# crowdbotp/socialways

Measured on AMD Instinct MI355X. Metric: GAN train steps/sec (256 scenes x 8 agents x 8+12 T per GPU step; fp32; social block on), higher is better.
Workload: dtype f32; 1 GPU; m1: 256 scenes x 8 agents x (8 obs + 12 pred) per GPU step = reference --batch-size 2048; use_social=True, n_unrolling_steps=1, info loss on; full=False, global_batch_scenes=256, parallelism=dp1, steps_per_graph_launch=32, settle_steps=992, rehearsal_regions=2, step_alg_bytes=5527040, inputs=z drawn on the host every step

## Files before the change

### socialways_amd/csrc/sw_disc.hip

```cpp
#include "../../include/socialways_hip.h"
#include "sw_lstm_dev.h"
#include "sw_wgrad.h"
#include "sw_wgrad_dev.h"
#include <cstdlib>
#ifdef SW_PHASE_STAMPS
__device__ long long sw_disc_stamps[16];
#define SW_STAMP(k) do { __builtin_amdgcn_sched_barrier(0); long long _t = clock64(); if (blockIdx.x == 0 && threadIdx.x == 0) sw_disc_stamps[k] += _t - _tprev; _tprev = _t; __builtin_amdgcn_sched_barrier(0); } while (0)
#define SW_STAMP_INIT long long _tprev = clock64()
extern "C" int sw_debug_disc_stamps(long long* out, int reset) {
  if (reset) { long long z[16] = {0}; return (int)hipMemcpyToSymbol(HIP_SYMBOL(sw_disc_stamps), z, sizeof(z)); }
  return (int)hipMemcpyFromSymbol(out, HIP_SYMBOL(sw_disc_stamps), 16 * sizeof(long long));
}
#else
#define SW_STAMP(k)
#define SW_STAMP_INIT
#endif

#define SW_DSTAMP(k) SW_STAMP(k)
#define SW_DSTAMP_INIT SW_STAMP_INIT
#include "sw_disc_dev.h"

__global__ __launch_bounds__(SW_THREADS, 2) void disc_fwd_kernel(
    const float* __restrict__ obsv, int To, int x_mode, const float* __restrict__ pred_a,
    const float* __restrict__ pred_b, int nb, const float* __restrict__ d_w, int B, int Tp, float* __restrict__ label_a, float* __restrict__ label_b,
// ... 231 lines not shown
  const bool live = (a0 + ln) < B;
  const int K4 = 4 * Tp, ldp = U.ldp;
  float* hw = smem + U.hw - F.of0;
  float* hwT = smem + U.hwT - T.of0T;

  float xpre[2][4];
  disc_xpre_load(xpre, pred_a, pred_b, a0, B, K4, ldp);
  const float tg0 = gl.targets[gl.t0], tg1 = gl.targets[gl.t1];
  const float z0 = gl.z[(size_t)b * SW_Z], z1 = gl.z[(size_t)b * SW_Z + 1];
  LstmW W;
  if (!obs_pre) disc_obs_operands(W, d_w, O, dimg);
  if (w_snap)
    for (int i = blockIdx.x * SW_THREADS + threadIdx.x; i < O.n; i += gridDim.x * SW_THREADS) w_snap[i] = d_w[i];
  disc_stage_heads(hw, F, d_w, O, K4, true);
  disc_stage_headT(hwT, T, true, nullptr, O, K4, dimg, false);
#pragma unroll
  for (int kk = 0; kk < 2; ++kk)
    disc_xpre_put(xpre, kk == 1, smem + U.x + kk * 16 * ldp, dsave + ds.px + (size_t)kk * B * K4, a0, B, K4, ldp);
  f32x4 c = {0.f, 0.f, 0.f, 0.f}, h = {0.f, 0.f, 0.f, 0.f};
  disc_seed_h(hbuf, obs_pre, dsave + ds.act, To, B, b);
  sw_barrier();
  const bool reg8 = !obs_pre && To == 8;
  f32x4 sg[8][4], sc[8];
  if (reg8) {
    float xa, xq;
    obs_x4_load(obsv, b, 0, 8, lg, xa, xq);
    asm volatile("" : "+v"(xa), "+v"(xq));
    float* hrow_g = dsave + ds.act + (size_t)b * 384 + 320 + u0 + 4 * lg;
    float* xrow = dsave + ds.x4s + (size_t)b * 4 + lg;
#pragma unroll
    for (int t = 0; t < 8; ++t) {
      const float xb = xa - (lg >= 2 ? xq : 0.f);
      obs_x4_load(obsv, b, t + 1 < 8 ? t + 1 : 7, 8, lg, xa, xq);
      lstm_cell(W, xb, &hbuf[(t & 1) * 16 * SW_HLD + ln * SW_HLD + 4 * lg], sg[t], c, h);
      sc[t] = c;
      st4(&hbuf[((t + 1) & 1) * 16 * SW_HLD + ln * SW_HLD + u0 + 4 * lg], h);
      st4g(hrow_g, h);
      *xrow = xb;
      hrow_g += (size_t)B * 384;
      xrow += (size_t)B * 4;
      sw_barrier();
      asm volatile("" : "+v"(xa), "+v"(xq));
    }
  } else if (!obs_pre) {
    lstm_obs_loop<0, true>(W, hbuf, obsv, To, B, b, c, h, dsave + ds.act, dsave + ds.x4s);
  }
  const float* hlast = &hbuf[(To & 1) * 16 * SW_HLD];

  const f32x4 o1reg = disc_obs_fc(hw, F, hlast, smem + U.o1, dsave + ds.o1 + (size_t)b * 32, live, smem + U.both, 2);
  float* xb_ = smem + U.x + br * 16 * ldp;
  float* q1_ = smem + U.q1 + br * 16 * LD32;
  float* both_ = smem + U.both + br * 16 * LD64;
  float* c1_ = smem + U.c1 + br * 16 * LD32;
  float* l1_ = smem + U.l1 + br * 16 * LD32;
  const size_t kb = (size_t)br * B + b;
  f32x4 q1reg, c1reg, l1reg;
  {
    const int m0 = 16 * wp;
    f32x4 acc = ld4(smem + U.bias + 2 * 32 + m0 + 4 * lg);
    acc = tile_mm_rt(hw + F.pe0 + (m0 + ln) * ldp + 4 * lg, xb_ + ln * ldp + 4 * lg, (ldp - 4) / 16, acc);
#pragma unroll
    for (int r = 0; r < 4; ++r) acc[r] = sw_lrelu(acc[r]);
    q1reg = acc;
    st4(q1_ + ln * LD32 + m0 + 4 * lg, acc);
    if (live) st4(dsave + ds.q1 + kb * 32 + m0 + 4 * lg, acc);
  }
  sw_barrier();
// ... 530 lines not shown
```

### socialways_amd/csrc/sw_lstm.hip

```cpp
#include "../../include/socialways_hip.h"
#include "sw_lstm_dev.h"
#include <cstdlib>

template <int XMODE, bool ACT, bool Y, bool X4S>
__global__ __launch_bounds__(SW_THREADS) void enc_lstm_fwd_kernel(
    const float* __restrict__ x, const float* __restrict__ enc_w, const float* __restrict__ h0,
    const float* __restrict__ c0, int B, int T, float* __restrict__ hT, float* __restrict__ cT,
    float* __restrict__ y, float* __restrict__ act, float* __restrict__ x4s, int t0, const float* __restrict__ aux_src,
    float* __restrict__ aux_dst, long long aux_n, const float* __restrict__ gimg) {
  const int tiles = (B + SW_TILE - 1) / SW_TILE;
  const int extra = (int)gridDim.x - tiles;
  if ((int)blockIdx.x < extra) {
    const long long n4 = aux_n >> 2, stride = (long long)extra * SW_THREADS;
    long long i = (long long)blockIdx.x * SW_THREADS + threadIdx.x;
    for (; i + 3 * stride < n4; i += 4 * stride) {
      const f32x4 v0 = ld4(aux_src + 4 * i), v1 = ld4(aux_src + 4 * (i + stride));
      const f32x4 v2 = ld4(aux_src + 4 * (i + 2 * stride)), v3 = ld4(aux_src + 4 * (i + 3 * stride));
      st4(aux_dst + 4 * i, v0);
      st4(aux_dst + 4 * (i + stride), v1);
      st4(aux_dst + 4 * (i + 2 * stride), v2);
      st4(aux_dst + 4 * (i + 3 * stride), v3);
    }
    for (; i < n4; i += stride) st4(aux_dst + 4 * i, ld4(aux_src + 4 * i));
    return;
  }
  constexpr int HS = ACT ? SW_ALD : SW_HLD, HO = ACT ? 320 : 0;
  __shared__ __attribute__((aligned(16))) float hbuf[2][SW_TILE * HS];
  __shared__ __attribute__((aligned(16))) float wx_lds[256 * 4];
  __shared__ __attribute__((aligned(16))) float bx_lds[256];
  const int lane = sw_lane(), wave = sw_wave(), ln = lane & 15, lg = lane >> 4;
  const int u0 = wave * 16;
  const int a0 = ((int)blockIdx.x - extra) * SW_TILE;
  const int b = min(a0 + ln, B - 1);
  LstmW W;
  if (gimg) {
    lstm_load_img(W, gimg, wave, lane);
  } else {
    lstm_load_whh(W, enc_w + swp::ENC_WHH, u0, ln, lg);
    lstm_prep_rows(enc_w + swp::ENC_EMB_W, enc_w + swp::ENC_EMB_B, enc_w + swp::ENC_WIH, enc_w + swp::ENC_BIH,
                   enc_w + swp::ENC_BHH, true, wx_lds, bx_lds);
  }
  f32x4 c = {0.f, 0.f, 0.f, 0.f}, h = {0.f, 0.f, 0.f, 0.f};
  if (h0) h = ld4(h0 + (size_t)b * 64 + u0 + 4 * lg);
  if (c0) c = ld4(c0 + (size_t)b * 64 + u0 + 4 * lg);
  st4(&hbuf[0][ln * HS + HO + u0 + 4 * lg], h);
  sw_barrier();
  if (!gimg) lstm_load_wx(W, wx_lds, bx_lds, u0, ln, lg);

  float xa, xq = 0.f;
  auto load_x = [&](int t) {
    if constexpr (XMODE == 0) obs_x4_load(x, b, t, T, lg, xa, xq);
    else xa = x[((size_t)b * T + t) * 4 + lg];
  };
  load_x(0);
  asm volatile("" : "+v"(xa), "+v"(xq));
  float* yrow = Y ? y + (size_t)b * T * 64 + u0 + 4 * lg : nullptr;
  float* xrow = X4S ? x4s + ((size_t)t0 * B + b) * 4 + lg : nullptr;
  for (int t = 0; t < T; ++t) {
    const float xb = XMODE == 0 ? xa - (lg >= 2 ? xq : 0.f) : xa;
    load_x(min(t + 1, T - 1));
    f32x4 gate[4];
    lstm_cell(W, xb, &hbuf[t & 1][ln * HS + HO + 4 * lg], gate, c, h);
    if constexpr (ACT) lstm_put_act_tile(hbuf[(t + 1) & 1], gate, c, h, ln, lg, u0);
    else st4(&hbuf[(t + 1) & 1][ln * HS + u0 + 4 * lg], h);
    if constexpr (Y) {
      st4(yrow, h);
      yrow += 64;
    }
    if constexpr (X4S) {
      *xrow = xb;
      xrow += (size_t)B * 4;
    }
    sw_barrier();
    if constexpr (ACT) lstm_store_act_tile(hbuf[(t + 1) & 1], act + (size_t)(t0 + t) * B * 384, a0, B, wave, lane);
    asm volatile("" : "+v"(xa), "+v"(xq));
  }
  st4(hT + (size_t)b * 64 + u0 + 4 * lg, h);
  st4(cT + (size_t)b * 64 + u0 + 4 * lg, c);
}

__global__ __launch_bounds__(512) void enc_lstm_fwd8_kernel(
    const float* __restrict__ x, const float* __restrict__ h0, const float* __restrict__ c0, int B, int T,
    float* __restrict__ hT, float* __restrict__ cT, float* __restrict__ act, float* __restrict__ x4s, int t0,
    const float* __restrict__ aux_src, float* __restrict__ aux_dst, long long aux_n, const float* __restrict__ gimg) {
  const int tiles = (B + SW_TILE - 1) / SW_TILE;
  const int extra = (int)gridDim.x - tiles;
  if ((int)blockIdx.x < extra) {
    const long long n4 = aux_n >> 2, stride = (long long)extra * 512;
    long long i = (long long)blockIdx.x * 512 + threadIdx.x;
    for (; i + stride < n4; i += 2 * stride) {
      const f32x4 v0 = ld4(aux_src + 4 * i), v1 = ld4(aux_src + 4 * (i + stride));
      st4(aux_dst + 4 * i, v0);
      st4(aux_dst + 4 * (i + stride), v1);
    }
    for (; i < n4; i += stride) st4(aux_dst + 4 * i, ld4(aux_src + 4 * i));
    return;
  }
  __shared__ __attribute__((aligned(16))) float hbuf[2][SW_TILE * SW_ALD];
  const int lane = sw_lane(), wave = sw_wave(), ln = lane & 15, lg = lane >> 4;
  const int ub = 8 * wave + 2 * lg;
  const int a0 = ((int)blockIdx.x - extra) * SW_TILE;
  const int b = min(a0 + ln, B - 1);
  f32x4 whh[2][4], bias[2];
  float wx[2];
#pragma unroll
  for (int tl = 0; tl < 2; ++tl) {
#pragma unroll
    for (int j = 0; j < 4; ++j) whh[tl][j] = ld4(gimg + swimg::OP_WHH8 + ((((size_t)wave * 2 + tl) * 4 + j) * 64 + lane) * 4);
    const int rowA = (2 * tl + ((ln & 3) >> 1)) * 64 + 8 * wave + 2 * (ln >> 2) + (ln & 1);
    wx[tl] = gimg[swimg::WX + rowA * 4 + lg];
#pragma unroll
    for (int r = 0; r < 4; ++r) bias[tl][r] = gimg[swimg::BX + (2 * tl + (r >> 1)) * 64 + ub + (r & 1)];
  }
  float2 c = {0.f, 0.f}, h = {0.f, 0.f};
  if (h0) h = *reinterpret_cast<const float2*>(h0 + (size_t)b * 64 + ub);
  if (c0) c = *reinterpret_cast<const float2*>(c0 + (size_t)b * 64 + ub);
  *reinterpret_cast<float2*>(&hbuf[0][ln * SW_ALD + 320 + ub]) = h;
  sw_barrier();
  float xa, xq = 0.f;
  obs_x4_load(x, b, 0, T, lg, xa, xq);
  asm volatile("" : "+v"(xa), "+v"(xq));
  float* xrow = x4s + ((size_t)t0 * B + b) * 4 + lg;
  for (int t = 0; t < T; ++t) {
    const float xb = xa - (lg >= 2 ? xq : 0.f);
    obs_x4_load(x, b, min(t + 1, T - 1), T, lg, xa, xq);
    const float* hrow = &hbuf[t & 1][ln * SW_ALD + 320 + 4 * lg];
    f32x4 bq[4];
#pragma unroll
    for (int j = 0; j < 4; ++j) bq[j] = ld4(hrow + 16 * j);
    f32x4 acc0 = SW_MFMA(wx[0], xb, bias[0]), acc1 = SW_MFMA(wx[1], xb, bias[1]);
#pragma unroll
    for (int j = 0; j < 4; ++j)
#pragma unroll
      for (int r = 0; r < 4; ++r) {
        acc0 = SW_MFMA(whh[0][j][r], bq[j][r], acc0);
        acc1 = SW_MFMA(whh[1][j][r], bq[j][r], acc1);
      }
    float2 gi, gf, gg, go;
#pragma unroll
    for (int e = 0; e < 2; ++e) {
      const float i_ = sw_sigmoid(acc0[e]), f_ = sw_sigmoid(acc0[2 + e]), g_ = sw_tanh(acc1[e]), o_ = sw_sigmoid(acc1[2 + e]);
      const float cp = e ? c.y : c.x;
      const float cn = fmaf(f_, cp, i_ * g_);
      const float hn = o_ * sw_tanh(cn);
      if (e) { gi.y = i_; gf.y = f_; gg.y = g_; go.y = o_; c.y = cn; h.y = hn; }
      else   { gi.x = i_; gf.x = f_; gg.x = g_; go.x = o_; c.x = cn; h.x = hn; }
    }
    float* row = &hbuf[(t + 1) & 1][ln * SW_ALD + ub];
    *reinterpret_cast<float2*>(row) = gi;
    *reinterpret_cast<float2*>(row + 64) = gf;
    *reinterpret_cast<float2*>(row + 128) = gg;
    *reinterpret_cast<float2*>(row + 192) = go;
    *reinterpret_cast<float2*>(row + 256) = c;
    *reinterpret_cast<float2*>(row + 320) = h;
    *xrow = xb;
    xrow += (size_t)B * 4;
    sw_barrier();
    {
      float* rows_t = act + (size_t)(t0 + t) * B * 384;
#pragma unroll
      for (int k = 0; k < 3; ++k) {
        const int f = k * 512 + (int)threadIdx.x, a = f / 96, c4 = f - a * 96;
        const f32x4 v = ld4(&hbuf[(t + 1) & 1][a * SW_ALD + 4 * c4]);
        st4g(rows_t + (size_t)min(a0 + a, B - 1) * 384 + 4 * c4, v);
      }
    }
    asm volatile("" : "+v"(xa), "+v"(xq));
  }
  *reinterpret_cast<float2*>(hT + (size_t)b * 64 + ub) = h;
  *reinterpret_cast<float2*>(cT + (size_t)b * 64 + ub) = c;
}

template <bool DY>
__global__ __launch_bounds__(SW_THREADS) void enc_lstm_bwd_kernel(
    const float* __restrict__ whh, const float* __restrict__ act, const float* __restrict__ c0,
    const float* __restrict__ dhT, const float* __restrict__ dcT, const float* __restrict__ dy, int B, int T,
    int t0, float* __restrict__ dgates, float* __restrict__ dh0, float* __restrict__ dc0, const float* __restrict__ gimg,
    const float* __restrict__ aux_src, float* __restrict__ aux_dst, const float* __restrict__ aux_mask, long long aux_n) {
  if (sw_aux_masked_copy(B, aux_src, aux_dst, aux_mask, aux_n)) return;
  __shared__ __attribute__((aligned(16))) float dgbuf[2][SW_TILE * SW_GLD];
  const int lane = sw_lane(), wave = sw_wave(), ln = lane & 15, lg = lane >> 4;
  const int u0 = wave * 16;
  const int a0 = blockIdx.x * SW_TILE;
  const int b = min(a0 + ln, B - 1);
  LstmWT W;
  lstm_load_whhT(W, gimg, swimg::OP_WHHT, whh, wave, lane);
  const float* act_b = act + ((size_t)t0 * B + b) * 384 + u0 + 4 * lg;
  f32x4 dh = ld4(dhT ? dhT + (size_t)b * 64 + u0 + 4 * lg : act_b);
  f32x4 dc = ld4(dcT ? dcT + (size_t)b * 64 + u0 + 4 * lg : act_b);
  if (!dhT) dh = f32x4{0.f, 0.f, 0.f, 0.f};
  if (!dcT) dc = f32x4{0.f, 0.f, 0.f, 0.f};
  const float* cstart = t0 > 0 ? act_b - (size_t)B * 384 + 256 : c0 ? c0 + (size_t)b * 64 + u0 + 4 * lg : nullptr;
  const LstmBptt S{act_b, cstart, dgbuf[0], dgates + ((size_t)t0 * B + a0) * 256, nullptr, a0, B};
  const float* dyp = DY ? dy + ((size_t)b * T + T - 1) * 64 + u0 + 4 * lg : nullptr;
  lstm_bptt_rows<true>(W, S, T, dh, dc, [&](f32x4& d) {
    if constexpr (DY) {
      d += ld4(dyp);
      dyp -= 64;
    }
  });
  if (dh0) st4(dh0 + (size_t)b * 64 + u0 + 4 * lg, dh);
// ... 156 lines not shown
```

### socialways_amd/csrc/sw_lstm_dev.h

```cpp
#pragma once
#include "sw_common.h"

#define SW_HLD 68
#define SW_GLD 260

struct LstmW {
  f32x4 whh[4][4];
  float wx[4];
  f32x4 bias[4];
};

__device__ __forceinline__ void lstm_prep_rows(const float* We, const float* be, const float* Wih,
                                               const float* bih, const float* bhh, bool composed,
                                               float* wx_lds, float* bx_lds) {
  int row = threadIdx.x;
  if (composed) {
    f32x4 w[16];
    const float* wr = Wih + (size_t)row * 64;
#pragma unroll
    for (int e = 0; e < 16; ++e) w[e] = ld4(wr + 4 * e);
    float a0 = 0.f, a1 = 0.f, a2 = 0.f, a3 = 0.f, ab = 0.f;
#pragma unroll
    for (int e = 0; e < 16; ++e) {
      f32x4 bq = ld4(be + 4 * e);
#pragma unroll
      for (int q = 0; q < 4; ++q) {
        f32x4 em = ld4(We + (4 * e + q) * 4);
        a0 = fmaf(w[e][q], em[0], a0);
        a1 = fmaf(w[e][q], em[1], a1);
        a2 = fmaf(w[e][q], em[2], a2);
        a3 = fmaf(w[e][q], em[3], a3);
        ab = fmaf(w[e][q], bq[q], ab);
      }
// ... 10 lines not shown
    wx_lds[row * 4 + 2] = w[2];
    wx_lds[row * 4 + 3] = w[3];
    bx_lds[row] = bih[row] + bhh[row];
  }
}

__device__ __forceinline__ void lstm_load_whh(LstmW& W, const float* Whh, int u0, int ln, int lg) {
#pragma unroll
  for (int g = 0; g < 4; ++g) {
    const float* wr = Whh + (size_t)(g * 64 + u0 + ln) * 64 + 4 * lg;
#pragma unroll
    for (int j = 0; j < 4; ++j) W.whh[g][j] = ld4(wr + 16 * j);
  }
}
__device__ __forceinline__ void lstm_load_wx(LstmW& W, const float* wx_lds, const float* bx_lds, int u0, int ln, int lg) {
#pragma unroll
  for (int g = 0; g < 4; ++g) {
    W.wx[g] = wx_lds[(g * 64 + u0 + ln) * 4 + lg];
    W.bias[g] = ld4(bx_lds + g * 64 + u0 + 4 * lg);
  }
}

__device__ __forceinline__ void lstm_load_img(LstmW& W, const float* __restrict__ gimg, int wave, int lane) {
  const int ln = lane & 15, lg = lane >> 4, u0 = wave * 16;
#pragma unroll
  for (int g = 0; g < 4; ++g) {
#pragma unroll
    for (int j = 0; j < 4; ++j) W.whh[g][j] = ld4(gimg + swimg::OP_WHH + ((((size_t)4 * g + wave) * 4 + j) * 64 + lane) * 4);
    W.wx[g] = gimg[swimg::WX + (g * 64 + u0 + ln) * 4 + lg];
    W.bias[g] = ld4(gimg + swimg::BX + g * 64 + u0 + 4 * lg);
  }
}

template <int NB>
__device__ __forceinline__ void lstm_products(const LstmW& W, const float (&xb)[NB], const float* const (&hrow)[NB],
                                              f32x4 (&acc)[NB][4]) {
  f32x4 b[NB][4];
#pragma unroll
  for (int k = 0; k < NB; ++k) {
#pragma unroll
    for (int j = 0; j < 4; ++j) b[k][j] = ld4(hrow[k] + 16 * j);
#pragma unroll
    for (int g = 0; g < 4; ++g) acc[k][g] = SW_MFMA(W.wx[g], xb[k], W.bias[g]);
  }
#pragma unroll
  for (int j = 0; j < 4; ++j) {
#pragma unroll
    for (int r = 0; r < 4; ++r) {
#pragma unroll
      for (int g = 0; g < 4; ++g) {
#pragma unroll
        for (int k = 0; k < NB; ++k) acc[k][g] = SW_MFMA(W.whh[g][j][r], b[k][j][r], acc[k][g]);
      }
    }
  }
}

__device__ __forceinline__ void lstm_gates(const f32x4 acc[4], f32x4 gate[4], f32x4& c, f32x4& h) {
#pragma unroll
  for (int r = 0; r < 4; ++r) {
    float i = sw_sigmoid(acc[0][r]);
    float f = sw_sigmoid(acc[1][r]);
    float g = sw_tanh(acc[2][r]);
    float o = sw_sigmoid(acc[3][r]);
    float cn = fmaf(f, c[r], i * g);
    gate[0][r] = i;
    gate[1][r] = f;
    gate[2][r] = g;
    gate[3][r] = o;
    c[r] = cn;
    h[r] = o * sw_tanh(cn);
  }
}

template <int NB>
__device__ __forceinline__ void lstm_cell(const LstmW& W, const float (&xb)[NB], const float* const (&hrow)[NB],
                                          f32x4 (&gate)[NB][4], f32x4 (&c)[NB], f32x4 (&h)[NB]) {
  f32x4 acc[NB][4];
  lstm_products<NB>(W, xb, hrow, acc);
#pragma unroll
  for (int k = 0; k < NB; ++k) lstm_gates(acc[k], gate[k], c[k], h[k]);
}
__device__ __forceinline__ void lstm_cell(const LstmW& W, float xb, const float* hrow, f32x4 gate[4],
                                          f32x4& c, f32x4& h) {
  f32x4 acc[1][4];
  lstm_products<1>(W, {xb}, {hrow}, acc);
  lstm_gates(acc[0], gate, c, h);
}

__device__ __forceinline__ void lstm_cell_bwd(const f32x4 gate[4], f32x4 ct, f32x4 cprev, f32x4 dh,
                                              f32x4& dc, f32x4 dgate[4]) {
#pragma unroll
  for (int r = 0; r < 4; ++r) {
    float i = gate[0][r], f = gate[1][r], g = gate[2][r], o = gate[3][r];
    float tc = sw_tanh(ct[r]);
    float d_o = dh[r] * tc;
    float dct = fmaf(dh[r] * o, 1.0f - tc * tc, dc[r]);
    dgate[0][r] = dct * g * i * (1.0f - i);
    dgate[1][r] = dct * cprev[r] * f * (1.0f - f);
    dgate[2][r] = dct * i * (1.0f - g * g);
    dgate[3][r] = d_o * o * (1.0f - o);
    dc[r] = dct * f;
  }
}

__device__ __forceinline__ void lstm_store_dgates_tile(const float* dgtile, float* __restrict__ rows ,
                                                       float* __restrict__ trash, int a0, int B, int wave, int lane) {
#pragma unroll
  for (int q = 0; q < 4; ++q) {
    const int a = 4 * wave + q;
    const f32x4 v = ld4(dgtile + a * SW_GLD + 4 * lane);
    float* dst = (a0 + a < B) ? rows + (size_t)a * 256 + 4 * lane
                 : trash      ? trash + a * 256 + 4 * lane
                              : rows + (size_t)(B - 1 - a0) * 256 + 4 * lane;
    st4g(dst, v);
  }
}

#define SW_ALD 388
// ... 116 lines not shown
    pre(dh);
  }
  lstm_bptt_step<false, false, DH0>(W, S, 0, gate, ct, cprev, dh, dc, stamp);
  stamp(11);
}

__device__ __forceinline__ void obs_x4_load(const float* pos, int b, int t, int T, int comp, float& a, float& q) {
  const float* p = pos + (size_t)b * T * 2;
  const int c = comp & 1, tt = t == 0 ? 1 : t;
  const bool vel = comp >= 2;
  a = p[(vel ? tt : t) * 2 + c];
  q = p[(vel ? tt - 1 : t) * 2 + c];
}
__device__ __forceinline__ float obs_x4(const float* pos, int b, int t, int T, int comp) {
  float a, q;
  obs_x4_load(pos, b, t, T, comp, a, q);
  return a - (comp >= 2 ? q : 0.f);
}

template <int XMODE, bool SAVE>
__device__ __forceinline__ void lstm_obs_loop(const LstmW& W, float* hbuf, const float* __restrict__ x, int T, int B, int b,
                                              f32x4& c, f32x4& h, float* __restrict__ act, float* __restrict__ x4s) {
  const int lane = sw_lane(), wave = sw_wave(), ln = lane & 15, lg = lane >> 4;
  const int u0 = wave * 16;
  float xa, xq = 0.f;
  auto load_x = [&](int t) {
    if constexpr (XMODE == 0) obs_x4_load(x, b, t, T, lg, xa, xq);
    else xa = x[((size_t)b * T + t) * 4 + lg];
  };
  load_x(0);
  asm volatile("" : "+v"(xa), "+v"(xq));
  float* arow = SAVE ? act + (size_t)b * 384 + u0 + 4 * lg : nullptr;
  float* xrow = SAVE ? x4s + (size_t)b * 4 + lg : nullptr;
  for (int t = 0; t < T; ++t) {
    const float xb = XMODE == 0 ? xa - (lg >= 2 ? xq : 0.f) : xa;
    load_x(min(t + 1, T - 1));
    f32x4 gate[4];
    lstm_cell(W, xb, &hbuf[(t & 1) * 16 * SW_HLD + ln * SW_HLD + 4 * lg], gate, c, h);
    st4(&hbuf[((t + 1) & 1) * 16 * SW_HLD + ln * SW_HLD + u0 + 4 * lg], h);
    if constexpr (SAVE) {
#pragma unroll
      for (int g = 0; g < 4; ++g) st4g(arow + g * 64, gate[g]);
      st4g(arow + 256, c);
      st4g(arow + 320, h);
      *xrow = xb;
      arow += (size_t)B * 384;
      xrow += (size_t)B * 4;
    }
    sw_barrier();
    asm volatile("" : "+v"(xa), "+v"(xq));
  }
}

__device__ __forceinline__ int obs_start(const int* __restrict__ obs_len, int b, int T, int xmode) {
  const int n = obs_len ? min(max(obs_len[b], xmode == 0 ? 2 : 1), T) : T;
  return T - n;
}
__device__ __forceinline__ void obs_x4_load_from(const float* pos, int b, int t, int s, int T, int comp, float& a, float& q) {
  const float* p = pos + (size_t)b * T * 2;
  const int c = comp & 1, te = max(t, s), tt = te == s ? s + 1 : te;
  const bool vel = comp >= 2;
  a = p[(vel ? tt : te) * 2 + c];
  q = p[(vel ? tt - 1 : te) * 2 + c];
}
template <int XMODE>
__device__ __forceinline__ void lstm_obs_loop_ragged(const LstmW& W, float* hbuf, const float* __restrict__ x, int T, int b, int s,
                                                     f32x4& c, f32x4& h) {
  const int lane = sw_lane(), wave = sw_wave(), ln = lane & 15, lg = lane >> 4;
  const int u0 = wave * 16;
  float xa, xq = 0.f;
  auto load_x = [&](int t) {
    if constexpr (XMODE == 0) obs_x4_load_from(x, b, t, s, T, lg, xa, xq);
    else xa = x[((size_t)b * T + max(t, s)) * 4 + lg];
  };
  load_x(0);
  asm volatile("" : "+v"(xa), "+v"(xq));
  for (int t = 0; t < T; ++t) {
    const float xb = XMODE == 0 ? xa - (lg >= 2 ? xq : 0.f) : xa;
    load_x(min(t + 1, T - 1));
    f32x4 gate[4];
    lstm_cell(W, xb, &hbuf[(t & 1) * 16 * SW_HLD + ln * SW_HLD + 4 * lg], gate, c, h);
    const bool on = t >= s;
#pragma unroll
    for (int r = 0; r < 4; ++r) {
// ... 29 lines not shown
```

### socialways_amd/csrc/sw_wgrad.hip

```cpp
#include "../../include/socialways_hip.h"
#include "sw_common.h"
#include "sw_wgrad.h"
#include "sw_wgrad_dev.h"
#include <stdlib.h>

__host__ __device__ inline int wg_grid_jobs(int total_jobs) { return (total_jobs + 31) & ~31; }
#ifdef SW_WG_STAMP
__device__ unsigned long long g_wg_stamps[4 * 4096];
extern "C" int sw_debug_wg_stamps(unsigned long long* host, int n) {
  return hipMemcpyFromSymbol(host, HIP_SYMBOL(g_wg_stamps), sizeof(unsigned long long) * (size_t)n) == hipSuccess ? 0 : -1;
}
#endif
__global__ __launch_bounds__(SW_THREADS, 2) void wgrad_partial_kernel(WgBatch batch, float* __restrict__ ws,
                                                                      const float* __restrict__ adam_step, double beta1,
                                                                      double beta2, float* __restrict__ bc_out) {
  __shared__ __attribute__((aligned(16))) float red[SW_WG_RED_FLOATS];
  if ((int)blockIdx.x >= wg_grid_jobs(batch.total_jobs)) {
    if (threadIdx.x == 0) {
      float bc1, bc2s;
      wg_adam_bc_compute(adam_step, beta1, beta2, bc1, bc2s);
      bc_out[0] = bc1;
      bc_out[1] = bc2s;
    }
    return;
// ... 67 lines not shown
  }
  float s = 0.f;
  float s1 = 0.f, s2 = 0.f, s3 = 0.f;
  int q = sub;
  for (; q + 3 * SW_WG_RSUB < P.nsplit; q += 4 * SW_WG_RSUB) {
    s += src[(size_t)q * stride];
    s1 += src[(size_t)(q + SW_WG_RSUB) * stride];
    s2 += src[(size_t)(q + 2 * SW_WG_RSUB) * stride];
    s3 += src[(size_t)(q + 3 * SW_WG_RSUB) * stride];
  }
  for (; q < P.nsplit; q += SW_WG_RSUB) s += src[(size_t)q * stride];
  s = (s + s1) + (s2 + s3);
#pragma unroll
  for (int o = SW_WG_REL; o < 64; o <<= 1) s += __shfl_xor(s, o);
  float bc1 = 1.f, bc2s = 1.f;
  if (ad.w) wg_adam_bc(ad, bc1, bc2s);
  if (!live || sub != 0) return;
  const float g = P.accumulate ? old1 + s : s;
  *dst = g;
  if (ad.w) wg_adam_fin(ad, a1, bc1, bc2s, g);
  if (dst2) {
    const float g2 = P.accumulate ? old2 + s : s;
    *dst2 = g2;
    if (ad.w) wg_adam_fin(ad, a2, bc1, bc2s, g2);
  }
}

bool wg_shape_ok(int N, int K) {
  for (int n0 = 0; n0 < N; n0 += 64)
    if (!wg_tiles(N - n0 < 64 ? N - n0 : 64, false)) return false;
  return K == 0 || wg_tiles(K, true) != 0;
}

int wg_add(WgBatch& b, const float* delta, int ldd, const float* act, int lda, int R, int N, int K, float* dW,
           int ldw, float* db, float* db2, int accumulate) {
  if (N > 256 || (ldd & 3) || (lda & 3)) return SW_ESHAPE;
  if ((long long)R * ldd >= (1LL << 31) || (long long)R * lda >= (1LL << 31)) return SW_ESHAPE;
  if (K < 1) return SW_ESHAPE;
  const int Nfull = N > 64 && (N & 63) && (N & 63) <= 32 && b.np + 2 * ((K + 63) / 64) <= SW_WG_MAXP ? (N & ~63) : N;
  for (int n0 = 0; n0 < N; n0 = (n0 == 0 ? Nfull : N)) {
    const int Nseg = n0 == 0 ? Nfull : N - Nfull;
    for (int c0 = 0; c0 < K; c0 += 64) {
      if (b.np >= SW_WG_MAXP) return SW_ESHAPE;
      const int c1 = c0 + 64 < K ? c0 + 64 : K;
      const bool has_ones = db && c1 == K;
      WgProblem& P = b.p[b.np++];
      P.delta = delta + n0; P.ldd = ldd; P.act = act + c0; P.lda = lda;
      P.R = R; P.N = Nseg; P.K = c1 - c0; P.ones = has_ones ? 1 : 0;
      P.dW = dW + (size_t)n0 * ldw + c0; P.ldw = ldw; P.db = has_ones ? db + n0 : nullptr;
      P.db2 = has_ones && db2 ? db2 + n0 : nullptr;
      P.accumulate = accumulate;
      P.pre = 0;
      P.act2 = nullptr; P.dW2 = nullptr; P.lda2 = P.ldw2 = P.K2 = P.row0 = 0;
      if (!wg_shape_ok(Nseg, P.K)) return SW_ESHAPE;
      P.nbn = (Nseg + 15) / 16;
      P.nbk = P.K > 0 ? wg_tiles(P.K, true) : 1;
    }
  }
  return SW_OK;
}

int wg_add_tail(WgBatch& b, const float* delta, int ldd, const float* act, int lda, int R, int N, int K, float* dW,
                int ldw, const float* act2, int lda2, int K2, float* dW2, int ldw2, int row0, float* db, float* db2,
                int accumulate) {
  if (N > 256 || (ldd & 3) || (lda & 3) || (lda2 & 3) || K != 64 || K2 != 4 || b.np >= SW_WG_MAXP)
    return SW_ESHAPE;
  if ((long long)R * ldd >= (1LL << 31) || (long long)R * lda >= (1LL << 31) || (long long)R * lda2 >= (1LL << 31)) return SW_ESHAPE;
  WgProblem& P = b.p[b.np++];
  P.delta = delta; P.ldd = ldd; P.act = act; P.lda = lda; P.R = R; P.N = N; P.K = K; P.ones = db ? 1 : 0;
  P.dW = dW; P.ldw = ldw; P.db = db; P.db2 = db ? db2 : nullptr; P.accumulate = accumulate; P.pre = 0;
  P.act2 = act2; P.lda2 = lda2; P.K2 = K2; P.dW2 = dW2; P.ldw2 = ldw2; P.row0 = row0;
  if (!wg_shape_ok(N, K)) return SW_ESHAPE;
  P.nbn = (N + 15) / 16;
  P.nbk = 4;
  return SW_OK;
}

int wg_add_pre(WgBatch& b, int N, int K, float* dW, int ldw, float* db, int nslices) {
  if (b.np >= SW_WG_MAXP || N < 1 || K < 1 || !db || nslices < 1) return SW_ESHAPE;
  WgProblem& P = b.p[b.np++];
  P.delta = nullptr; P.act = nullptr; P.ldd = P.lda = 0; P.R = 0;
  P.N = N; P.K = K; P.ones = 1; P.dW = dW; P.ldw = ldw; P.db = db; P.db2 = nullptr; P.accumulate = 0;
  P.nbn = (N + 15) / 16; P.nbk = (K + 1 + 15) / 16;
  P.act2 = nullptr; P.dW2 = nullptr; P.lda2 = P.ldw2 = P.K2 = P.row0 = 0;
  P.pre = nslices;
  b.top_reserved += (size_t)nslices * N * (K + 1);
  if (b.top_reserved > SW_WG_WS_FLOATS) return SW_ESHAPE;
  P.ws_off = SW_WG_WS_FLOATS - b.top_reserved;
  return SW_OK;
}

#ifndef SW_WG_GROUP_C0
#define SW_WG_GROUP_C0 256.0
#endif
#ifndef SW_WG_ROUND_UP
#define SW_WG_ROUND_UP 0.75
#endif
static double wg_cost(const WgProblem& P) {
  double c = 0;
  for (int n0 = 0; n0 < P.N; n0 += 64) {
// ... 121 lines not shown
```

### socialways_amd/csrc/sw_wgrad_dev.h

```cpp
#pragma once
#include <type_traits>
#include "sw_common.h"
#include "sw_wgrad.h"
#ifndef SW_WG_DEPTH
#define SW_WG_DEPTH 4
#endif
#ifndef SW_WG_DEPTH5
#define SW_WG_DEPTH5 2
#endif
#ifndef SW_WG_DEPTH_TAIL
#define SW_WG_DEPTH_TAIL SW_WG_DEPTH
#endif

#define SW_WG_RLD 69

template <int NV>
__device__ __forceinline__ void wg_ldv(float (&v)[NV], const float* p) {
  if constexpr (NV == 4) {
    const f32x4 q = *reinterpret_cast<const f32x4*>(p);
    v[0] = q[0]; v[1] = q[1]; v[2] = q[2]; v[3] = q[3];
  } else if constexpr (NV == 3) {
    struct __attribute__((packed, aligned(4))) P3 { float a, b, c; };
    const P3 q = *reinterpret_cast<const P3*>(p);
    v[0] = q.a; v[1] = q.b; v[2] = q.c;
  } else if constexpr (NV == 2) {
    const float2 q = *reinterpret_cast<const float2*>(p);
    v[0] = q.x; v[1] = q.y;
  } else {
    v[0] = p[0];
  }
}

__host__ __device__ inline int wg_tiles(int n, bool allow3) {
  if (n <= 16) return 1;
  for (int t = (n + 15) >> 4; t <= 4; ++t)
    if ((t != 3 || allow3) && n % t == 0) return t;
  return 0;
}

template <int NA, int KR, int K2, int ONES, int DSCALE = 1>
__device__ __forceinline__ void wg_run(const float* __restrict__ dbase, const float* __restrict__ abase, int ldd, int lda,
                                       int rbeg, int rend, int rmax, int acol, int bcol, int lg, int ln,
                                       float* __restrict__ mine,
                                       const float* __restrict__ abase2, int lda2, int row0, int xoff) {
  constexpr int KT = KR, XC = K2 + ONES;
  f32x4 acc[NA][KT];
#pragma unroll
  for (int i = 0; i < NA; ++i) {
#pragma unroll
    for (int kt = 0; kt < KT; ++kt) acc[i][kt] = f32x4{0.f, 0.f, 0.f, 0.f};
  }
  float xacc[NA][XC > 0 ? XC : 1];
#pragma unroll
  for (int i = 0; i < NA; ++i) {
#pragma unroll
    for (int c = 0; c < (XC > 0 ? XC : 1); ++c) xacc[i][c] = 0.f;
  }
  constexpr int DEPTH = (K2 > 0 ? SW_WG_DEPTH_TAIL : SW_WG_DEPTH) * DSCALE;
  float a[DEPTH][NA], b[DEPTH][KT];
  f32x4 xq[DEPTH];
  auto load = [&](int r0, float (&av)[NA], float (&bv)[KT], f32x4& xv) {
    const int rc = min(r0 + lg, rmax);
    wg_ldv<NA>(av, dbase + (unsigned)(rc * ldd + acol));
    if constexpr (K2 > 0) {
      wg_ldv<KR>(bv, abase + (unsigned)(max(rc, row0) * lda + bcol));
      xv = ld4(abase2 + (unsigned)(rc * lda2));
    } else {
      wg_ldv<KR>(bv, abase + (unsigned)(rc * lda + bcol));
    }
  };
#pragma unroll
  for (int q = 0; q < DEPTH - 1; ++q) load(rbeg + 4 * q, a[q], b[q], xq[q]);
  for (int r = rbeg; r < rend; r += 4 * DEPTH) {
#pragma unroll
    for (int q = 0; q < DEPTH; ++q) {
      load(r + 4 * (q + DEPTH - 1), a[(q + DEPTH - 1) % DEPTH], b[(q + DEPTH - 1) % DEPTH], xq[(q + DEPTH - 1) % DEPTH]);
      asm volatile("" ::: "memory");
#pragma unroll
      for (int i = 0; i < NA; ++i) asm volatile("" : "+v"(a[q][i]));
#pragma unroll
      for (int kt = 0; kt < KT; ++kt) asm volatile("" : "+v"(b[q][kt]));
      if constexpr (K2 > 0) asm volatile("" : "+v"(xq[q]));
      const int rr = r + 4 * q + lg;
      const float rs = rr < rend ? 1.0f : 0.0f;
      float av[NA], bv[KT];
#pragma unroll
      for (int i = 0; i < NA; ++i) av[i] = a[q][i] * rs;
      if constexpr (K2 > 0) {
        const float rs0 = rr >= row0 ? 1.0f : 0.0f;
#pragma unroll
        for (int kt = 0; kt < KR; ++kt) bv[kt] = b[q][kt] * rs0;
      } else {
#pragma unroll
        for (int kt = 0; kt < KR; ++kt) bv[kt] = b[q][kt];
      }
#pragma unroll
      for (int i = 0; i < NA; ++i) {
#pragma unroll
        for (int kt = 0; kt < KT; ++kt) {
          acc[i][kt] = SW_MFMA(av[i], bv[kt], acc[i][kt]);
        }
      }
#pragma unroll
      for (int i = 0; i < NA; ++i) {
        if constexpr (K2 > 0) {
#pragma unroll
          for (int c = 0; c < K2; ++c) xacc[i][c] = fmaf(av[i], xq[q][c], xacc[i][c]);
        }
        if constexpr (ONES) xacc[i][K2] += av[i];
      }
    }
  }
#pragma unroll
  for (int i = 0; i < NA; ++i) {
#pragma unroll
    for (int kt = 0; kt < KT; ++kt) {
#pragma unroll
      for (int r = 0; r < 4; ++r) {
        const int orow = NA * (4 * lg + r) + i;
        if (KR * ln + kt < xoff) mine[orow * SW_WG_RLD + KR * ln + kt] = acc[i][kt][r];
      }
    }
  }
  if constexpr (XC > 0) {
#pragma unroll
    for (int i = 0; i < NA; ++i) {
#pragma unroll
      for (int c = 0; c < XC; ++c) {
        float v = xacc[i][c];
        v += __shfl_xor(v, 16);
        v += __shfl_xor(v, 32);
        if (lg == 0) mine[(NA * ln + i) * SW_WG_RLD + xoff + c] = v;
      }
    }
  }
}

#define SW_WG_RED_FLOATS (4 * 64 * SW_WG_RLD)
template <int DSCALE = 1>
__device__ __forceinline__ void wg_job(const WgBatch& batch, float* __restrict__ ws, int job, float* red) {
  const int lane = sw_lane(), wave = sw_wave(), ln = lane & 15, lg = lane >> 4;
  int p = 0;
#pragma unroll 1
  while (p + 1 < batch.np && job >= batch.job0s[p + 1]) ++p;
  const WgProblem& P = batch.p[p];
  const int j = job - P.job0;
  const int NB = (P.N + 63) >> 6;
  const int sg = j / NB, nb = j - sg * NB;
  const int s = sg * 4 + wave;
  const int N = P.N, K = P.K, Kc = P.K + P.K2 + P.ones;
  const int n0 = nb * 64;
  const int Nb = min(64, N - n0);
  const int NA = wg_tiles(Nb, false);
  const int KR = K > 0 ? wg_tiles(K, true) : 1;
  const int nsub = P.nsplit * 4;
  const int rows_per = (((P.R + nsub - 1) / nsub) + 3) & ~3;
  const int rbeg = min(P.R, s * rows_per);
  const int rend = min(P.R, rbeg + rows_per);
  const int acol = n0 + max(0, min(NA * ln, Nb - NA));
  const int bcol = max(0, min(KR * ln, K - KR));
  float* mine = red + wave * 64 * SW_WG_RLD;
#define WG_CASE(na, kr, k2, on)                                                                                     \
  case ((na * 8 + kr) * 2 + (k2 ? 1 : 0)) * 2 + on:                                                                 \
    wg_run<na, kr, k2, on, DSCALE>(P.delta, P.act, P.ldd, P.lda, rbeg, rend, P.R - 1, acol, bcol, lg, ln,              \
                                   mine, P.act2 ? P.act2 : P.delta, P.act2 ? P.lda2 : P.ldd, P.row0, K);            \
    break;
#define WG_CASES(na)                                                                                                \
  WG_CASE(na, 1, 0, 0) WG_CASE(na, 2, 0, 0) WG_CASE(na, 3, 0, 0) WG_CASE(na, 4, 0, 0)                               \
  WG_CASE(na, 1, 0, 1) WG_CASE(na, 2, 0, 1) WG_CASE(na, 3, 0, 1) WG_CASE(na, 4, 0, 1)                               \
  WG_CASE(na, 4, 4, 0) WG_CASE(na, 4, 4, 1)
  switch (((NA * 8 + KR) * 2 + (P.K2 ? 1 : 0)) * 2 + (P.ones ? 1 : 0)) {
    WG_CASES(1) WG_CASES(2) WG_CASES(4)
  }
#undef WG_CASES
#undef WG_CASE
  sw_barrier();
  float* out = ws + P.ws_off + (size_t)sg * N * Kc;
  const int rows = min(64, N - n0), cols = min(SW_WG_RLD, Kc);
  const int dq = SW_THREADS / cols, dr = SW_THREADS - dq * cols;
  int rr = threadIdx.x / cols, cc = threadIdx.x - rr * cols;
  const float* r0 = red, *r1 = red + 64 * SW_WG_RLD, *r2 = red + 2 * 64 * SW_WG_RLD, *r3 = red + 3 * 64 * SW_WG_RLD;
  for (int e = threadIdx.x; e < rows * cols; e += SW_THREADS) {
    const int o = rr * SW_WG_RLD + cc;
    const float v = (r0[o] + r1[o]) + (r2[o] + r3[o]);
    out[(size_t)(n0 + rr) * Kc + cc] = v;
    cc += dr;
    rr += dq;
    if (cc >= cols) {
      cc -= cols;
      ++rr;
    }
  }
}
```

Baseline: 2753 steps/s.

## Skip recurrent matmul at zero initial state and use buffer loads in wgrad

The first LSTM step of the encoder, discriminator and generic obs loops now skips the hidden-state LDS reads and the W_hh MFMA chain when the initial hidden state is known to be zero. Separately, the weight-gradient inner loop now uses raw buffer loads with per-range descriptors. Out-of-range rows read as zero, which removes the per-row clamp and masking multiplies. The host-side span checks are updated to fit the descriptor byte limits. The risk is correctness at range edges, since masking now relies on the buffer bounds and on row0 handling through the descriptor base.

```diff
diff --git a/socialways_amd/csrc/sw_disc.hip b/socialways_amd/csrc/sw_disc.hip
--- a/socialways_amd/csrc/sw_disc.hip
+++ b/socialways_amd/csrc/sw_disc.hip
@@ -287,7 +287,9 @@
     for (int t = 0; t < 8; ++t) {
       const float xb = xa - (lg >= 2 ? xq : 0.f);
       obs_x4_load(obsv, b, t + 1 < 8 ? t + 1 : 7, 8, lg, xa, xq);
-      lstm_cell(W, xb, &hbuf[(t & 1) * 16 * SW_HLD + ln * SW_HLD + 4 * lg], sg[t], c, h);
+      const float* hrow = &hbuf[(t & 1) * 16 * SW_HLD + ln * SW_HLD + 4 * lg];
+      if (t == 0) lstm_cell<false>(W, xb, hrow, sg[t], c, h);
+      else lstm_cell(W, xb, hrow, sg[t], c, h);
       sc[t] = c;
       st4(&hbuf[((t + 1) & 1) * 16 * SW_HLD + ln * SW_HLD + u0 + 4 * lg], h);
       st4g(hrow_g, h);
diff --git a/socialways_amd/csrc/sw_lstm.hip b/socialways_amd/csrc/sw_lstm.hip
--- a/socialways_amd/csrc/sw_lstm.hip
+++ b/socialways_amd/csrc/sw_lstm.hip
@@ -56,11 +56,11 @@
   asm volatile("" : "+v"(xa), "+v"(xq));
   float* yrow = Y ? y + (size_t)b * T * 64 + u0 + 4 * lg : nullptr;
   float* xrow = X4S ? x4s + ((size_t)t0 * B + b) * 4 + lg : nullptr;
-  for (int t = 0; t < T; ++t) {
+  auto step = [&](int t, auto hp) {
     const float xb = XMODE == 0 ? xa - (lg >= 2 ? xq : 0.f) : xa;
     load_x(min(t + 1, T - 1));
     f32x4 gate[4];
-    lstm_cell(W, xb, &hbuf[t & 1][ln * HS + HO + 4 * lg], gate, c, h);
+    lstm_cell<decltype(hp)::value>(W, xb, &hbuf[t & 1][ln * HS + HO + 4 * lg], gate, c, h);
     if constexpr (ACT) lstm_put_act_tile(hbuf[(t + 1) & 1], gate, c, h, ln, lg, u0);
     else st4(&hbuf[(t + 1) & 1][ln * HS + u0 + 4 * lg], h);
     if constexpr (Y) {
@@ -74,7 +74,10 @@
     sw_barrier();
     if constexpr (ACT) lstm_store_act_tile(hbuf[(t + 1) & 1], act + (size_t)(t0 + t) * B * 384, a0, B, wave, lane);
     asm volatile("" : "+v"(xa), "+v"(xq));
-  }
+  };
+  if (h0) step(0, std::true_type{});
+  else step(0, std::false_type{});
+  for (int t = 1; t < T; ++t) step(t, std::true_type{});
   st4(hT + (size_t)b * 64 + u0 + 4 * lg, h);
   st4(cT + (size_t)b * 64 + u0 + 4 * lg, c);
 }
@@ -121,21 +124,23 @@
   obs_x4_load(x, b, 0, T, lg, xa, xq);
   asm volatile("" : "+v"(xa), "+v"(xq));
   float* xrow = x4s + ((size_t)t0 * B + b) * 4 + lg;
-  for (int t = 0; t < T; ++t) {
+  auto step = [&](int t, auto hp) {
     const float xb = xa - (lg >= 2 ? xq : 0.f);
     obs_x4_load(x, b, min(t + 1, T - 1), T, lg, xa, xq);
-    const float* hrow = &hbuf[t & 1][ln * SW_ALD + 320 + 4 * lg];
-    f32x4 bq[4];
-#pragma unroll
-    for (int j = 0; j < 4; ++j) bq[j] = ld4(hrow + 16 * j);
     f32x4 acc0 = SW_MFMA(wx[0], xb, bias[0]), acc1 = SW_MFMA(wx[1], xb, bias[1]);
-#pragma unroll
-    for (int j = 0; j < 4; ++j)
-#pragma unroll
-      for (int r = 0; r < 4; ++r) {
-        acc0 = SW_MFMA(whh[0][j][r], bq[j][r], acc0);
-        acc1 = SW_MFMA(whh[1][j][r], bq[j][r], acc1);
-      }
+    if constexpr (decltype(hp)::value) {
+      const float* hrow = &hbuf[t & 1][ln * SW_ALD + 320 + 4 * lg];
+      f32x4 bq[4];
+#pragma unroll
+      for (int j = 0; j < 4; ++j) bq[j] = ld4(hrow + 16 * j);
+#pragma unroll
+      for (int j = 0; j < 4; ++j)
+#pragma unroll
+        for (int r = 0; r < 4; ++r) {
+          acc0 = SW_MFMA(whh[0][j][r], bq[j][r], acc0);
+          acc1 = SW_MFMA(whh[1][j][r], bq[j][r], acc1);
+        }
+    }
     float2 gi, gf, gg, go;
 #pragma unroll
     for (int e = 0; e < 2; ++e) {
@@ -166,7 +171,10 @@
       }
     }
     asm volatile("" : "+v"(xa), "+v"(xq));
-  }
+  };
+  if (h0) step(0, std::true_type{});
+  else step(0, std::false_type{});
+  for (int t = 1; t < T; ++t) step(t, std::true_type{});
   *reinterpret_cast<float2*>(hT + (size_t)b * 64 + ub) = h;
   *reinterpret_cast<float2*>(cT + (size_t)b * 64 + ub) = c;
 }
diff --git a/socialways_amd/csrc/sw_lstm_dev.h b/socialways_amd/csrc/sw_lstm_dev.h
--- a/socialways_amd/csrc/sw_lstm_dev.h
+++ b/socialways_amd/csrc/sw_lstm_dev.h
@@ -1,4 +1,5 @@
 #pragma once
+#include <type_traits>
 #include "sw_common.h"
 
 #define SW_HLD 68
@@ -75,25 +76,29 @@
   }
 }
 
-template <int NB>
+template <int NB, bool HP = true>
 __device__ __forceinline__ void lstm_products(const LstmW& W, const float (&xb)[NB], const float* const (&hrow)[NB],
                                               f32x4 (&acc)[NB][4]) {
   f32x4 b[NB][4];
 #pragma unroll
   for (int k = 0; k < NB; ++k) {
-#pragma unroll
-    for (int j = 0; j < 4; ++j) b[k][j] = ld4(hrow[k] + 16 * j);
+    if constexpr (HP) {
+#pragma unroll
+      for (int j = 0; j < 4; ++j) b[k][j] = ld4(hrow[k] + 16 * j);
+    }
 #pragma unroll
     for (int g = 0; g < 4; ++g) acc[k][g] = SW_MFMA(W.wx[g], xb[k], W.bias[g]);
   }
-#pragma unroll
-  for (int j = 0; j < 4; ++j) {
-#pragma unroll
-    for (int r = 0; r < 4; ++r) {
-#pragma unroll
-      for (int g = 0; g < 4; ++g) {
-#pragma unroll
-        for (int k = 0; k < NB; ++k) acc[k][g] = SW_MFMA(W.whh[g][j][r], b[k][j][r], acc[k][g]);
+  if constexpr (HP) {
+#pragma unroll
+    for (int j = 0; j < 4; ++j) {
+#pragma unroll
+      for (int r = 0; r < 4; ++r) {
+#pragma unroll
+        for (int g = 0; g < 4; ++g) {
+#pragma unroll
+          for (int k = 0; k < NB; ++k) acc[k][g] = SW_MFMA(W.whh[g][j][r], b[k][j][r], acc[k][g]);
+        }
       }
     }
   }
@@ -124,10 +129,11 @@
 #pragma unroll
   for (int k = 0; k < NB; ++k) lstm_gates(acc[k], gate[k], c[k], h[k]);
 }
+template <bool HP = true>
 __device__ __forceinline__ void lstm_cell(const LstmW& W, float xb, const float* hrow, f32x4 gate[4],
                                           f32x4& c, f32x4& h) {
   f32x4 acc[1][4];
-  lstm_products<1>(W, {xb}, {hrow}, acc);
+  lstm_products<1, HP>(W, {xb}, {hrow}, acc);
   lstm_gates(acc[0], gate, c, h);
 }
 
@@ -310,11 +316,11 @@
   asm volatile("" : "+v"(xa), "+v"(xq));
   float* arow = SAVE ? act + (size_t)b * 384 + u0 + 4 * lg : nullptr;
   float* xrow = SAVE ? x4s + (size_t)b * 4 + lg : nullptr;
-  for (int t = 0; t < T; ++t) {
+  auto step = [&](int t, auto hp) {
     const float xb = XMODE == 0 ? xa - (lg >= 2 ? xq : 0.f) : xa;
     load_x(min(t + 1, T - 1));
     f32x4 gate[4];
-    lstm_cell(W, xb, &hbuf[(t & 1) * 16 * SW_HLD + ln * SW_HLD + 4 * lg], gate, c, h);
+    lstm_cell<decltype(hp)::value>(W, xb, &hbuf[(t & 1) * 16 * SW_HLD + ln * SW_HLD + 4 * lg], gate, c, h);
     st4(&hbuf[((t + 1) & 1) * 16 * SW_HLD + ln * SW_HLD + u0 + 4 * lg], h);
     if constexpr (SAVE) {
 #pragma unroll
@@ -327,7 +333,9 @@
     }
     sw_barrier();
     asm volatile("" : "+v"(xa), "+v"(xq));
-  }
+  };
+  step(0, std::false_type{});
+  for (int t = 1; t < T; ++t) step(t, std::true_type{});
 }
 
 __device__ __forceinline__ int obs_start(const int* __restrict__ obs_len, int b, int T, int xmode) {
diff --git a/socialways_amd/csrc/sw_wgrad.hip b/socialways_amd/csrc/sw_wgrad.hip
--- a/socialways_amd/csrc/sw_wgrad.hip
+++ b/socialways_amd/csrc/sw_wgrad.hip
@@ -123,10 +123,15 @@
   return K == 0 || wg_tiles(K, true) != 0;
 }
 
+static bool wg_span_ok(int R, int ld, int row0) {
+  const long long rows = (long long)R / 4 + 4 + 8 * 4 * SW_WG_DEPTH + row0;
+  return rows * ld * 4 < (1LL << 31);
+}
+
 int wg_add(WgBatch& b, const float* delta, int ldd, const float* act, int lda, int R, int N, int K, float* dW,
            int ldw, float* db, float* db2, int accumulate) {
   if (N > 256 || (ldd & 3) || (lda & 3)) return SW_ESHAPE;
-  if ((long long)R * ldd >= (1LL << 31) || (long long)R * lda >= (1LL << 31)) return SW_ESHAPE;
+  if (!wg_span_ok(R, ldd, 0) || !wg_span_ok(R, lda, 0)) return SW_ESHAPE;
   if (K < 1) return SW_ESHAPE;
   const int Nfull = N > 64 && (N & 63) && (N & 63) <= 32 && b.np + 2 * ((K + 63) / 64) <= SW_WG_MAXP ? (N & ~63) : N;
   for (int n0 = 0; n0 < N; n0 = (n0 == 0 ? Nfull : N)) {
@@ -156,7 +161,7 @@
                 int accumulate) {
   if (N > 256 || (ldd & 3) || (lda & 3) || (lda2 & 3) || K != 64 || K2 != 4 || b.np >= SW_WG_MAXP)
     return SW_ESHAPE;
-  if ((long long)R * ldd >= (1LL << 31) || (long long)R * lda >= (1LL << 31) || (long long)R * lda2 >= (1LL << 31)) return SW_ESHAPE;
+  if (row0 < 0 || !wg_span_ok(R, ldd, 0) || !wg_span_ok(R, lda, row0) || !wg_span_ok(R, lda2, 0)) return SW_ESHAPE;
   WgProblem& P = b.p[b.np++];
   P.delta = delta; P.ldd = ldd; P.act = act; P.lda = lda; P.R = R; P.N = N; P.K = K; P.ones = db ? 1 : 0;
   P.dW = dW; P.ldw = ldw; P.db = db; P.db2 = db ? db2 : nullptr; P.accumulate = accumulate; P.pre = 0;
diff --git a/socialways_amd/csrc/sw_wgrad_dev.h b/socialways_amd/csrc/sw_wgrad_dev.h
--- a/socialways_amd/csrc/sw_wgrad_dev.h
+++ b/socialways_amd/csrc/sw_wgrad_dev.h
@@ -14,21 +14,27 @@
 
 #define SW_WG_RLD 69
 
+typedef __amdgpu_buffer_rsrc_t wg_rsrc;
+__device__ __forceinline__ wg_rsrc wg_make_rsrc(const float* base, unsigned bytes) {
+  return __builtin_amdgcn_make_buffer_rsrc(const_cast<float*>(base), 0, (int)bytes, 0x00020000);
+}
 template <int NV>
-__device__ __forceinline__ void wg_ldv(float (&v)[NV], const float* p) {
+__device__ __forceinline__ void wg_ldv(float (&v)[NV], wg_rsrc rs, unsigned off) {
+  unsigned u[NV];
   if constexpr (NV == 4) {
-    const f32x4 q = *reinterpret_cast<const f32x4*>(p);
-    v[0] = q[0]; v[1] = q[1]; v[2] = q[2]; v[3] = q[3];
+    const auto q = __builtin_amdgcn_raw_buffer_load_b128(rs, (int)off, 0, 0);
+    u[0] = q[0]; u[1] = q[1]; u[2] = q[2]; u[3] = q[3];
   } else if constexpr (NV == 3) {
-    struct __attribute__((packed, aligned(4))) P3 { float a, b, c; };
-    const P3 q = *reinterpret_cast<const P3*>(p);
-    v[0] = q.a; v[1] = q.b; v[2] = q.c;
+    const auto q = __builtin_amdgcn_raw_buffer_load_b96(rs, (int)off, 0, 0);
+    u[0] = q[0]; u[1] = q[1]; u[2] = q[2];
   } else if constexpr (NV == 2) {
-    const float2 q = *reinterpret_cast<const float2*>(p);
-    v[0] = q.x; v[1] = q.y;
+    const auto q = __builtin_amdgcn_raw_buffer_load_b64(rs, (int)off, 0, 0);
+    u[0] = q[0]; u[1] = q[1];
   } else {
-    v[0] = p[0];
+    u[0] = __builtin_amdgcn_raw_buffer_load_b32(rs, (int)off, 0, 0);
   }
+#pragma unroll
+  for (int i = 0; i < NV; ++i) v[i] = __uint_as_float(u[i]);
 }
 
 __host__ __device__ inline int wg_tiles(int n, bool allow3) {
@@ -40,7 +46,7 @@
 
 template <int NA, int KR, int K2, int ONES, int DSCALE = 1>
 __device__ __forceinline__ void wg_run(const float* __restrict__ dbase, const float* __restrict__ abase, int ldd, int lda,
-                                       int rbeg, int rend, int rmax, int acol, int bcol, int lg, int ln,
+                                       int rbeg, int rend, int acol, int bcol, int lg, int ln,
                                        float* __restrict__ mine,
                                        const float* __restrict__ abase2, int lda2, int row0, int xoff) {
   constexpr int KT = KR, XC = K2 + ONES;
@@ -59,55 +65,51 @@
   constexpr int DEPTH = (K2 > 0 ? SW_WG_DEPTH_TAIL : SW_WG_DEPTH) * DSCALE;
   float a[DEPTH][NA], b[DEPTH][KT];
   f32x4 xq[DEPTH];
-  auto load = [&](int r0, float (&av)[NA], float (&bv)[KT], f32x4& xv) {
-    const int rc = min(r0 + lg, rmax);
-    wg_ldv<NA>(av, dbase + (unsigned)(rc * ldd + acol));
+  const int abeg = K2 > 0 ? max(rbeg, row0) : rbeg, aend = max(abeg, rend);
+  const wg_rsrc drs = wg_make_rsrc(dbase + (size_t)rbeg * ldd, (unsigned)(rend - rbeg) * (unsigned)ldd * 4u);
+  const wg_rsrc ars = wg_make_rsrc(abase + (size_t)abeg * lda, (unsigned)(aend - abeg) * (unsigned)lda * 4u);
+  const wg_rsrc xrs = wg_make_rsrc(abase2 + (size_t)rbeg * lda2, (unsigned)(rend - rbeg) * (unsigned)lda2 * 4u);
+  unsigned doff = (unsigned)(lg * ldd + acol) * 4u, aoff = (unsigned)((rbeg - abeg + lg) * lda + bcol) * 4u;
+  unsigned xoff2 = (unsigned)(lg * lda2) * 4u;
+  const unsigned dstep = 16u * (unsigned)ldd, astep = 16u * (unsigned)lda, xstep = 16u * (unsigned)lda2;
+  auto load = [&](float (&av)[NA], float (&bv)[KT], f32x4& xv) {
+    wg_ldv<NA>(av, drs, doff);
+    doff += dstep;
+    wg_ldv<KR>(bv, ars, aoff);
+    aoff += astep;
     if constexpr (K2 > 0) {
-      wg_ldv<KR>(bv, abase + (unsigned)(max(rc, row0) * lda + bcol));
-      xv = ld4(abase2 + (unsigned)(rc * lda2));
-    } else {
-      wg_ldv<KR>(bv, abase + (unsigned)(rc * lda + bcol));
+      float x4[4];
+      wg_ldv<4>(x4, xrs, xoff2);
+      xv = f32x4{x4[0], x4[1], x4[2], x4[3]};
+      xoff2 += xstep;
     }
   };
 #pragma unroll
-  for (int q = 0; q < DEPTH - 1; ++q) load(rbeg + 4 * q, a[q], b[q], xq[q]);
+  for (int q = 0; q < DEPTH - 1; ++q) load(a[q], b[q], xq[q]);
   for (int r = rbeg; r < rend; r += 4 * DEPTH) {
 #pragma unroll
     for (int q = 0; q < DEPTH; ++q) {
-      load(r + 4 * (q + DEPTH - 1), a[(q + DEPTH - 1) % DEPTH], b[(q + DEPTH - 1) % DEPTH], xq[(q + DEPTH - 1) % DEPTH]);
+      load(a[(q + DEPTH - 1) % DEPTH], b[(q + DEPTH - 1) % DEPTH], xq[(q + DEPTH - 1) % DEPTH]);
       asm volatile("" ::: "memory");
 #pragma unroll
       for (int i = 0; i < NA; ++i) asm volatile("" : "+v"(a[q][i]));
 #pragma unroll
       for (int kt = 0; kt < KT; ++kt) asm volatile("" : "+v"(b[q][kt]));
       if constexpr (K2 > 0) asm volatile("" : "+v"(xq[q]));
-      const int rr = r + 4 * q + lg;
-      const float rs = rr < rend ? 1.0f : 0.0f;
-      float av[NA], bv[KT];
-#pragma unroll
-      for (int i = 0; i < NA; ++i) av[i] = a[q][i] * rs;
-      if constexpr (K2 > 0) {
-        const float rs0 = rr >= row0 ? 1.0f : 0.0f;
-#pragma unroll
-        for (int kt = 0; kt < KR; ++kt) bv[kt] = b[q][kt] * rs0;
-      } else {
-#pragma unroll
-        for (int kt = 0; kt < KR; ++kt) bv[kt] = b[q][kt];
-      }
 #pragma unroll
       for (int i = 0; i < NA; ++i) {
 #pragma unroll
         for (int kt = 0; kt < KT; ++kt) {
-          acc[i][kt] = SW_MFMA(av[i], bv[kt], acc[i][kt]);
+          acc[i][kt] = SW_MFMA(a[q][i], b[q][kt], acc[i][kt]);
         }
       }
 #pragma unroll
       for (int i = 0; i < NA; ++i) {
         if constexpr (K2 > 0) {
 #pragma unroll
-          for (int c = 0; c < K2; ++c) xacc[i][c] = fmaf(av[i], xq[q][c], xacc[i][c]);
+          for (int c = 0; c < K2; ++c) xacc[i][c] = fmaf(a[q][i], xq[q][c], xacc[i][c]);
         }
-        if constexpr (ONES) xacc[i][K2] += av[i];
+        if constexpr (ONES) xacc[i][K2] += a[q][i];
       }
     }
   }
@@ -155,14 +157,14 @@
   const int KR = K > 0 ? wg_tiles(K, true) : 1;
   const int nsub = P.nsplit * 4;
   const int rows_per = (((P.R + nsub - 1) / nsub) + 3) & ~3;
-  const int rbeg = min(P.R, s * rows_per);
-  const int rend = min(P.R, rbeg + rows_per);
+  const int rbeg = __builtin_amdgcn_readfirstlane(min(P.R, s * rows_per));
+  const int rend = __builtin_amdgcn_readfirstlane(min(P.R, rbeg + rows_per));
   const int acol = n0 + max(0, min(NA * ln, Nb - NA));
   const int bcol = max(0, min(KR * ln, K - KR));
   float* mine = red + wave * 64 * SW_WG_RLD;
 #define WG_CASE(na, kr, k2, on)                                                                                     \
   case ((na * 8 + kr) * 2 + (k2 ? 1 : 0)) * 2 + on:                                                                 \
-    wg_run<na, kr, k2, on, DSCALE>(P.delta, P.act, P.ldd, P.lda, rbeg, rend, P.R - 1, acol, bcol, lg, ln,              \
+    wg_run<na, kr, k2, on, DSCALE>(P.delta, P.act, P.ldd, P.lda, rbeg, rend, acol, bcol, lg, ln,                      \
                                    mine, P.act2 ? P.act2 : P.delta, P.act2 ? P.lda2 : P.ldd, P.row0, K);            \
     break;
 #define WG_CASES(na)                                                                                                \
```

Result: faster. 2815 steps/s, median of 6 (+2.2%).
